# TrackieWay-OSS/TrackieLLM

Measured on AMD Instinct MI355X. Metric: cortex cycles/sec (frame+1s audio+128 tok), higher is better.
Workload: dtype int8 x q4_K/q6_K (i32 acc, f32 scales); 1 GPU; configs[3] fused cycle: YOLOv8n 640x640 frame (preprocess+network+NMS) + 1 s PCM (VAD + Whisper-tiny.en log-mel/encoder/16 forced decoder steps) + Mistral-7B Q4_K_M 64-token prefill and 128-token greedy decode, 3 concurrent HIP streams; concurrent_cycles_per_gpu=768, decode_groups=3, rows_per_llm_pass=256, layers=32, parallelism=replicas x1

## Files before the change

### trackiellm_amd/csrc/llm/tk_llm_kernels.hip

```cpp
#include "tk_llm_kernels.h"

#include "../common/tk_exact_math.h"
#include <stdio.h>
#include <stdlib.h>

#include <atomic>

#include "../common/tk_ggml_blocks.h"
#include "../common/tk_sample_device.h"

typedef int v4i __attribute__((ext_vector_type(4)));
typedef int v2i __attribute__((ext_vector_type(2)));
typedef float v4f __attribute__((ext_vector_type(4)));
typedef float v2f __attribute__((ext_vector_type(2)));

#define TK_WAVE 64

__global__ void k_synth_blocks(int type, uint64_t seed, uint64_t tid, int64_t nblocks, float scale, uint8_t* out) {
    int64_t b = (int64_t)blockIdx.x * blockDim.x + threadIdx.x;
    if (b >= nblocks) return;
    float x[256];
    for (int i = 0; i < 256; ++i) x[i] = scale * tk_synth_normal(seed, tid, (uint64_t)(256 * b + i));
    if (type == TK_TYPE_Q4_K) {
        tk_block_q4_K blk;
// ... 1436 lines not shown
    }
}

static int tk_num_cu() {
    static std::atomic<int> cached[64];
    int dev = 0;
    if (hipGetDevice(&dev) != hipSuccess || dev < 0 || dev >= 64) return 256;
    int v = cached[dev].load(std::memory_order_relaxed);
    if (v == 0) {
        int n = 0;
        v = (hipDeviceGetAttribute(&n, hipDeviceAttributeMultiprocessorCount, dev) == hipSuccess && n > 0) ? n : 256;
        cached[dev].store(v, std::memory_order_relaxed);
    }
    return v;
}
#define TK_NUM_CU tk_num_cu()

#define TK_MAX_DYN_LDS (160 * 1024)
#include <mutex>
template <typename F>
static hipError_t opt_in_lds(F* fn) { return hipFuncSetAttribute((const void*)fn, hipFuncAttributeMaxDynamicSharedMemorySize, TK_MAX_DYN_LDS); }

static constexpr int TK_GEMM32_FROM_ROWS = 12 * TK_ROW_SLOTS + 1;

typedef void (*TkGemvKernel)(TkGemvArgs, int, int);
typedef void (*TkGemm32Kernel)(TkGemvArgs, int, int, int);
static const TkGemvKernel k_gemv_fns[3][2][2][4] = {
    {{{k_gemv_w4a8<1, 1, 1, 0>, k_gemv_w4a8<1, 1, 2, 0>, k_gemv_w4a8<1, 1, 3, 0>, k_gemv_w4a8<1, 1, 4, 0>},
      {k_gemv_w4a8<2, 1, 1, 0>, k_gemv_w4a8<2, 1, 2, 0>, k_gemv_w4a8<2, 1, 3, 0>, k_gemv_w4a8<2, 1, 4, 0>}},
     {{k_gemv_w4a8<1, 2, 1, 0>, nullptr, k_gemv_w4a8<1, 2, 3, 0>, k_gemv_w4a8<1, 2, 4, 0>},
      {k_gemv_w4a8<2, 2, 1, 0>, nullptr, k_gemv_w4a8<2, 2, 3, 0>, k_gemv_w4a8<2, 2, 4, 0>}}},
    {{{}, {k_gemv_w4a8<2, 1, 1, 1>, k_gemv_w4a8<2, 1, 2, 1>, k_gemv_w4a8<2, 1, 3, 1>, k_gemv_w4a8<2, 1, 4, 1>}}},
    {{{}, {k_gemv_w4a8<2, 1, 1, 2>, k_gemv_w4a8<2, 1, 2, 2>, k_gemv_w4a8<2, 1, 3, 2>, k_gemv_w4a8<2, 1, 4, 2>}}},
};
static const TkGemvKernel k_gemm_fns[5][4] = {
    {k_gemm_w4a8<4, 1>, k_gemm_w4a8<4, 2>, k_gemm_w4a8<4, 3>, k_gemm_w4a8<4, 4>},     {k_gemm_w4a8<6, 1>, k_gemm_w4a8<6, 2>, k_gemm_w4a8<6, 3>, k_gemm_w4a8<6, 4>},
    {k_gemm_w4a8<8, 1>, k_gemm_w4a8<8, 2>, k_gemm_w4a8<8, 3>, k_gemm_w4a8<8, 4>},     {k_gemm_w4a8<10, 1>, k_gemm_w4a8<10, 2>, k_gemm_w4a8<10, 3>, k_gemm_w4a8<10, 4>},
    {k_gemm_w4a8<12, 1>, k_gemm_w4a8<12, 2>, k_gemm_w4a8<12, 3>, k_gemm_w4a8<12, 4>},
};
static const TkGemm32Kernel k_gemm32_fns[4] = {k_gemm32_w4a8<1>, k_gemm32_w4a8<2>, k_gemm32_w4a8<3>, k_gemm32_w4a8<4>};

void tk_launch_gemv(const TkGemvArgs& a, hipStream_t s) {
    int types = 0;
    for (int i = 0; i < a.nseg; ++i) types |= a.seg[i].type == TK_TYPE_Q4_K ? 1 : a.seg[i].type == TK_TYPE_Q5_K ? 4 : 2;
    if ((types & 4) && types != 4) {
        int i0 = 0, col = a.col0;
        while (i0 < a.nseg) {
            int i1 = i0 + 1;
            while (i1 < a.nseg && a.seg[i1].type == a.seg[i0].type) ++i1;
            TkGemvArgs p = a;
            p.nseg = i1 - i0;
            for (int i = 0; i < p.nseg; ++i) p.seg[i] = a.seg[i0 + i];
            p.col0 = col;
            tk_launch_gemv(p, s);
            for (int i = i0; i < i1; ++i) col += a.seg[i].row_tiles * TK_TILE_ROWS;
            i0 = i1;
        }
        return;
    }
    const int ti = types == 4 ? 3 : types - 1;
    int row_tiles = 0;
    for (int i = 0; i < a.nseg; ++i) row_tiles += a.seg[i].row_tiles;
    int groups = TK_NUM_CU / a.ks;
    if (groups < 1) groups = 1;
    if (groups > row_tiles) groups = row_tiles;
    int waves = (row_tiles + groups - 1) / groups;
    while (waves > 8) { groups *= 2; waves = (row_tiles + groups - 1) / groups; }
    if (a.nrows >= TK_GEMM32_FROM_ROWS) {
        const int pairs = a.swiglu ? a.seg[0].row_tiles : row_tiles / 2;
        const int g32 = (pairs + 3) / 4;
        const int n_halves = a.nrows > 8 * TK_ROW_SLOTS ? 2 : 1;
        const size_t ldsb = (size_t)2 * TK_G32_MT * TK_RING_TILE_BYTES;
        hipLaunchKernelGGL(k_gemm32_fns[ti], dim3(g32 * a.ks * n_halves), dim3(256), ldsb, s, a, g32, row_tiles, n_halves);
        return;
    }
    if (a.nrows > 2 * TK_ROW_SLOTS) {
        const int mtb = a.nrows > 10 * TK_ROW_SLOTS ? 12 : a.nrows > 8 * TK_ROW_SLOTS ? 10 : a.nrows > 6 * TK_ROW_SLOTS ? 8 : a.nrows > 4 * TK_ROW_SLOTS ? 6 : 4;
        const size_t ldsb = (size_t)2 * mtb * TK_RING_TILE_BYTES;
        hipLaunchKernelGGL(k_gemm_fns[mtb / 2 - 2][ti], dim3(groups * a.ks), dim3(64 * waves), ldsb, s, a, groups, row_tiles);
        return;
    }
    const int mt = a.nrows > TK_ROW_SLOTS ? 2 : 1;
    const size_t lds = tk_gemv_lds_bytes(a.K, a.ks, mt);
    const int nb = a.K / a.ks / 256;
    const int gti = mt == 2 && types == 2 ? 2 : ti;
    const int pf = nb % 2 == 0 ? 2 : 1;
    const size_t fuse_lds = a.fuse == 1 ? ((size_t)a.K + 4) * sizeof(float) : 0;
    const int fuse = a.fuse && mt == 1 && pf == 2 ? (a.fuse == 1 ? 1 : 2) : 0;
    hipLaunchKernelGGL(k_gemv_fns[fuse][mt - 1][pf - 1][gti], dim3(groups * a.ks), dim3(64 * waves), lds + fuse_lds, s, a, groups, row_tiles);
}

bool tk_gemv_fuses_producer(int nrows, int K, int ks, int fks) {
    return nrows >= 1 && nrows <= TK_GEMV_FUSE_MAX_ROWS && ks >= 1 && K % (512 * ks) == 0 && fks >= 0 && fks <= TK_RMS_MAX_KS;
}

__device__ __forceinline__ float sum_partials(const float* partial, int ks, int n_total, int row, int col) {
    float o = partial[(int64_t)row * n_total + col];
    for (int s = 1; s < ks; ++s) o = o + partial[((int64_t)s * TK_MAX_ROWS + row) * n_total + col];
    return o;
}

__global__ void k_qkv_rope_append(const float* partial, int ks, int n_total, int n_head, int n_kv_head, int head_dim, const float* rope_cos,
                                  const float* rope_sin, const int32_t* seq, const int32_t* pos, float* qbuf, uint16_t* kcache,
                                  uint16_t* vcache, int layer, int max_seq, int max_ctx) {
    const int kvh = blockIdx.x, r = blockIdx.y;
    const int half = head_dim / 2, grp = n_head / n_kv_head;
    const int QD = n_head * head_dim, KVD = n_kv_head * head_dim;
    const int p = pos[r], sq = seq[r];
    const float* cs = rope_cos + (int64_t)p * half;
    const float* sn = rope_sin + (int64_t)p * half;
    const int64_t cbase = ((((int64_t)layer * max_seq + sq) * n_kv_head + kvh) * max_ctx + p) * head_dim;
    for (int idx = threadIdx.x; idx < (grp + 1) * half; idx += blockDim.x) {
        const int hsel = idx / half, i = idx % half;
        if (hsel < grp) {
            const int col = (kvh * grp + hsel) * head_dim + 2 * i;
            const float a = sum_partials(partial, ks, n_total, r, col);
            const float b = sum_partials(partial, ks, n_total, r, col + 1);
            qbuf[(int64_t)r * QD + col] = tk_fmaf(-b, sn[i], a * cs[i]);
            qbuf[(int64_t)r * QD + col + 1] = tk_fmaf(a, sn[i], b * cs[i]);
        } else {
            const int col = QD + kvh * head_dim + 2 * i;
            const float a = sum_partials(partial, ks, n_total, r, col);
            const float b = sum_partials(partial, ks, n_total, r, col + 1);
            kcache[cbase + 2 * i] = tk_f32_to_f16(tk_fmaf(-b, sn[i], a * cs[i]));
            kcache[cbase + 2 * i + 1] = tk_f32_to_f16(tk_fmaf(a, sn[i], b * cs[i]));
            const int vcol = QD + KVD + kvh * head_dim + 2 * i;
            vcache[cbase + 2 * i] = tk_f32_to_f16(sum_partials(partial, ks, n_total, r, vcol));
            vcache[cbase + 2 * i + 1] = tk_f32_to_f16(sum_partials(partial, ks, n_total, r, vcol + 1));
        }
    }
}

void tk_launch_qkv_rope_append(const float* partial, int ks, int n_total, int n_head, int n_kv_head, int head_dim, const float* rope_cos,
                               const float* rope_sin, const int32_t* seq, const int32_t* pos, int nrows, float* qbuf, uint16_t* kcache,
                               uint16_t* vcache, int layer, int max_seq, int max_ctx, hipStream_t s) {
    hipLaunchKernelGGL(k_qkv_rope_append, dim3(n_kv_head, nrows), dim3(256), 0, s, partial, ks, n_total, n_head, n_kv_head, head_dim, rope_cos,
                       rope_sin, seq, pos, qbuf, kcache, vcache, layer, max_seq, max_ctx);
}

#define TK_ATT_MAX_GRP 4
#define TK_ATT_TSPLIT 4
__device__ __forceinline__ float sum_partials_wide(const float* partial, int ks, int n_total, int row, int col) {
    float p[TK_RMS_MAX_KS];
#pragma unroll
    for (int s = 0; s < TK_RMS_MAX_KS; ++s)
        if (s < ks) p[s] = partial[((int64_t)s * TK_MAX_ROWS + row) * n_total + col];
    float o = p[0];
#pragma unroll
    for (int s = 1; s < TK_RMS_MAX_KS; ++s)
        if (s < ks) o = o + p[s];
    return o;
}

__device__ __forceinline__ void att_stage(const uint16_t* run, int row0, int last_row, int rb , uint8_t* slot, bool swz, int wave, int lane, int chunk,
                                          int row_end = -1) {
    const int pieces = chunk * rb / 1024, ppr = rb / 16;
    for (int pc = wave; pc < pieces; pc += 4) {
        if (row_end >= 0 && row0 + pc * 64 / ppr >= row_end) continue;
        const int idx = pc * 64 + lane;
        const int r = idx / ppr, cs = idx % ppr;
        int gr = row0 + r;
        gr = gr < last_row ? gr : last_row;
        const int src = swz ? (cs ^ (r & (ppr - 1))) : cs;
        const auto gs = (const __attribute__((address_space(1))) void*)((const uint8_t*)run + (int64_t)gr * rb + src * 16);
        const auto ls = (__attribute__((address_space(3))) void*)(slot + pc * 1024);
        __builtin_amdgcn_global_load_lds(gs, ls, 16, 0, 0);
    }
}

template <int GQ, bool FUSED, int HD , int CH >
__global__ __launch_bounds__(256, 1) void k_attention(const float* __restrict__ qbuf, const float* __restrict__ partial, int ks, int n_total,
                                                    const float* __restrict__ rope_cos, const float* __restrict__ rope_sin,
                                                    uint16_t* __restrict__ kcache, uint16_t* __restrict__ vcache, const int32_t* __restrict__ seq,
                                                    const int32_t* __restrict__ pos, int n_head, int n_kv_head, int head_dim_rt, int layer, int max_seq,
                                                    int max_ctx, TkActQ8 out) {
    extern __shared__ __attribute__((aligned(16))) uint8_t att_lds[];
    const int head_dim = HD ? HD : head_dim_rt;
    const int hb = blockIdx.x, r = blockIdx.y, t = threadIdx.x, lane = t & 63;
    const int kvh = hb * GQ / (n_head / n_kv_head);
    const int wave = __builtin_amdgcn_readfirstlane(t >> 6);
    const int p = pos[r], T = p + 1, sq = seq[r];
    const int W = GQ * head_dim;
    const int rb = head_dim * 2;
    const int half = head_dim / 2, QD = n_head * head_dim, KVD = n_kv_head * head_dim;
    const int slot_bytes = CH * rb;
    uint8_t* ring = att_lds;
    float* qs = (float*)(att_lds + 2 * slot_bytes);
    float* sc = qs + W;
    float* red = sc + (size_t)GQ * max_ctx;
    uint16_t* own = (uint16_t*)(red + 4 * TK_ATT_MAX_GRP);
    float* part = (float*)ring;
    float* lpart = part + TK_ATT_TSPLIT * W;
    float* obuf = lpart + TK_ATT_TSPLIT * TK_ATT_MAX_GRP;
    const int64_t run0 = (((int64_t)layer * max_seq + sq) * n_kv_head + kvh) * (int64_t)max_ctx * head_dim;
    const uint16_t* krun = kcache + run0;
    const uint16_t* vrun = vcache + run0;
    const int nchunk = (T + CH - 1) / CH;
    const int total = 2 * nchunk;
    const int last_row = max_ctx - 1;
    const int ppr = rb / 16;
    auto issue = [&](int j) {
        const bool is_k = j < nchunk;
        const int c = is_k ? j : j - nchunk;
        att_stage(is_k ? krun : vrun, c * CH, last_row, rb, ring + (j % 2) * slot_bytes, is_k, wave, lane, CH, CH > 64 ? T : -1);
    };
    const int ppw = slot_bytes / 4096;
    auto acquire = [&](int j) {
        const int ahead = total - 1 - j < 0 ? total - 1 - j : 0;
        wait_vmcnt(ahead * ppw);
        __syncthreads();
        if (j + 1 < total) issue(j + 1);
    };

    for (int j = 0; j < 1 && j < total; ++j) issue(j);
    if (FUSED) {
        const float* cs = rope_cos + (int64_t)p * half;
        const float* sn = rope_sin + (int64_t)p * half;
        for (int idx = t; idx < (GQ + 2) * half; idx += 256) {
            const int hsel = idx / half, i = idx % half;
            if (hsel < GQ) {
                const int col = (hb * GQ + hsel) * head_dim + 2 * i;
                const float a = sum_partials_wide(partial, ks, n_total, r, col), b = sum_partials_wide(partial, ks, n_total, r, col + 1);
                qs[hsel * head_dim + 2 * i] = tk_fmaf(-b, sn[i], a * cs[i]);
                qs[hsel * head_dim + 2 * i + 1] = tk_fmaf(a, sn[i], b * cs[i]);
            } else if (hsel == GQ) {
                const int col = QD + kvh * head_dim + 2 * i;
                const float a = sum_partials_wide(partial, ks, n_total, r, col), b = sum_partials_wide(partial, ks, n_total, r, col + 1);
                const uint16_t k0 = tk_f32_to_f16(tk_fmaf(-b, sn[i], a * cs[i])), k1 = tk_f32_to_f16(tk_fmaf(a, sn[i], b * cs[i]));
                const uint32_t kk = (uint32_t)k0 | ((uint32_t)k1 << 16);
                *(uint32_t*)(kcache + run0 + (int64_t)p * head_dim + 2 * i) = kk;
                *(uint32_t*)(own + 2 * i) = kk;
            } else {
                const int col = QD + KVD + kvh * head_dim + 2 * i;
                const uint16_t v0 = tk_f32_to_f16(sum_partials_wide(partial, ks, n_total, r, col)), v1 = tk_f32_to_f16(sum_partials_wide(partial, ks, n_total, r, col + 1));
                const uint32_t vv = (uint32_t)v0 | ((uint32_t)v1 << 16);
                *(uint32_t*)(vcache + run0 + (int64_t)p * head_dim + 2 * i) = vv;
                *(uint32_t*)(own + head_dim + 2 * i) = vv;
            }
        }
    } else {
        for (int i = t; i < W; i += 256) qs[i] = qbuf[(int64_t)r * QD + hb * W + i];
    }
    const float att_scale = tk_divf(1.0f, tk_sqrtf((float)head_dim));

    float mx = -INFINITY;
    for (int c = 0; c < nchunk; ++c) {
        acquire(c);
        uint8_t* slot = ring + (c % 2) * slot_bytes;
        if (FUSED && c == nchunk - 1) {
            const int rr = p - c * CH;
            if (t < ppr) *(uint4*)(slot + rr * rb + ((t ^ (rr & (ppr - 1))) * 16)) = *(const uint4*)((const uint8_t*)own + t * 16);
            __syncthreads();
        }
        for (int idx = t; idx < GQ * CH; idx += 256) {
            const int h = idx / CH, rr = idx % CH, tt = c * CH + rr;
            if (tt < T) {
                const uint8_t* kr = slot + rr * rb;
                const float* qh = qs + h * head_dim;
                float a = 0.0f;
                constexpr int KB = HD ? HD / 8 : 1;
                for (int i0 = 0; i0 < ppr; i0 += KB) {
                    uint4 kv[KB];
#pragma unroll
                    for (int u = 0; u < KB; ++u) kv[u] = *(const uint4*)(kr + (((i0 + u) ^ (rr & (ppr - 1))) * 16));
#pragma unroll
                    for (int u = 0; u < KB; ++u) {
                        const v4f q0 = *(const v4f*)(qh + 8 * (i0 + u)), q1 = *(const v4f*)(qh + 8 * (i0 + u) + 4);
                        const uint32_t kw[4] = {kv[u].x, kv[u].y, kv[u].z, kv[u].w};
#pragma unroll
                        for (int e = 0; e < 8; ++e) {
                            const float kf = f16bits_to_f32((kw[e >> 1] >> (16 * (e & 1))) & 0xffffu);
                            a = tk_fmaf(e < 4 ? q0[e] : q1[e - 4], kf, a);
                        }
                    }
                }
                const float s = a * att_scale;
                sc[(size_t)h * max_ctx + tt] = s;
                mx = tk_fmaxf(mx, s);
            }
        }
    }
    if (CH <= 64) {
        float m = mx;
        for (int s = CH / 2; s >= 1; s >>= 1) m = tk_fmaxf(m, wave_xor_f(m, s));
        if ((lane & (CH - 1)) == 0 && t < GQ * CH) red[t / CH] = m;
    } else {
        float m = mx;
        for (int s = 32; s >= 1; s >>= 1) m = tk_fmaxf(m, wave_xor_f(m, s));
        if (lane == 0) red[TK_ATT_MAX_GRP + wave] = m;
    }
    __syncthreads();
    if (CH > 64 && t < GQ) {
        float m = red[TK_ATT_MAX_GRP + t * (CH / 64)];
        for (int w = 1; w < CH / 64; ++w) m = tk_fmaxf(m, red[TK_ATT_MAX_GRP + t * (CH / 64) + w]);
        red[t] = m;
    }
    if (CH > 64) __syncthreads();
    for (int h = 0; h < GQ; ++h) {
        const float m = red[h];
        for (int tt = t; tt < T; tt += 256) sc[(size_t)h * max_ctx + tt] = tk_expf(sc[(size_t)h * max_ctx + tt] - m);
    }
    float acc[GQ][2][2], l[GQ];
#pragma unroll
    for (int h = 0; h < GQ; ++h) { l[h] = 0.0f; acc[h][0][0] = acc[h][0][1] = acc[h][1][0] = acc[h][1][1] = 0.0f; }
    for (int c = 0; c < nchunk; ++c) {
        acquire(nchunk + c);
        uint8_t* slot = ring + ((nchunk + c) % 2) * slot_bytes;
        if (FUSED && c == nchunk - 1) {
            const int rr = p - c * CH;
            if (t < ppr) *(uint4*)(slot + rr * rb + t * 16) = *(const uint4*)((const uint8_t*)(own + head_dim) + t * 16);
            __syncthreads();
        }
        const int t_end = T - c * CH < CH ? T - c * CH : CH;
        constexpr int PB = 4;
        for (int rr0 = wave; rr0 < t_end; rr0 += PB * TK_ATT_TSPLIT) {
            float pr[PB][GQ];
            uint32_t vv[PB][2];
#pragma unroll
            for (int u = 0; u < PB; ++u) {
                const int rr = rr0 + u * TK_ATT_TSPLIT;
                const bool live = rr < t_end;
                const int rc = live ? rr : t_end - 1;
#pragma unroll
                for (int h = 0; h < GQ; ++h) pr[u][h] = live ? sc[(size_t)h * max_ctx + c * CH + rc] : 0.0f;
#pragma unroll
                for (int db = 0; db < 2; ++db) {
                    const int d0 = 2 * lane + 128 * db;
                    vv[u][db] = d0 < head_dim ? *(const uint32_t*)(slot + rc * rb + d0 * 2) : 0u;
                }
            }
#pragma unroll
            for (int u = 0; u < PB; ++u) {
#pragma unroll
                for (int db = 0; db < 2; ++db) {
                    if (2 * lane + 128 * db < head_dim) {
                        const float v0 = f16bits_to_f32(vv[u][db] & 0xffffu), v1 = f16bits_to_f32(vv[u][db] >> 16);
#pragma unroll
                        for (int h = 0; h < GQ; ++h) {
                            acc[h][db][0] = tk_fmaf(pr[u][h], v0, acc[h][db][0]);
                            acc[h][db][1] = tk_fmaf(pr[u][h], v1, acc[h][db][1]);
                        }
                    }
                }
#pragma unroll
                for (int h = 0; h < GQ; ++h) l[h] = l[h] + pr[u][h];
            }
        }
    }
    __syncthreads();
#pragma unroll
    for (int h = 0; h < GQ; ++h) {
#pragma unroll
        for (int db = 0; db < 2; ++db) {
            const int d0 = 2 * lane + 128 * db;
            if (d0 < head_dim) {
                part[wave * W + h * head_dim + d0] = acc[h][db][0];
                part[wave * W + h * head_dim + d0 + 1] = acc[h][db][1];
            }
        }
        if (lane == 0) lpart[wave * TK_ATT_MAX_GRP + h] = l[h];
    }
    __syncthreads();
    for (int i = t; i < W; i += 256) {
        const int h = i / head_dim;
        const float a = ((part[i] + part[W + i]) + part[2 * W + i]) + part[3 * W + i];
        const float ll = ((lpart[h] + lpart[TK_ATT_MAX_GRP + h]) + lpart[2 * TK_ATT_MAX_GRP + h]) + lpart[3 * TK_ATT_MAX_GRP + h];
        obuf[i] = tk_divf(a, ll);
    }
    __syncthreads();
    for (int c = t; c < W / 8; c += 256) {
        float v[8];
#pragma unroll
        for (int i = 0; i < 8; ++i) v[i] = obuf[8 * c + i];
        quantize_chunk8(v, hb * (W / 8) + c, r, out);
    }
}

__global__ __launch_bounds__(1024) void k_attention_narrow(const float* __restrict__ partial, int ks, int n_total, const float* __restrict__ rope_cos,
                                                            const float* __restrict__ rope_sin, uint16_t* __restrict__ kcache, uint16_t* __restrict__ vcache,
                                                            const int32_t* __restrict__ seq, const int32_t* __restrict__ pos, int n_head, int n_kv_head, int layer,
                                                            int max_seq, int max_ctx, int cap, TkActQ8 out) {
    extern __shared__ __attribute__((aligned(16))) uint8_t att_lds[];
    constexpr int HD = 128, GQ = 2, W = GQ * HD, RB = HD * 2, PPR = RB / 16;
    const int hb = blockIdx.x, r = blockIdx.y, t = threadIdx.x, lane = t & 63;
    const int wave = __builtin_amdgcn_readfirstlane(t >> 6);
    const int kvh = hb * GQ / (n_head / n_kv_head);
    const int p = pos[r], T = p + 1, sq = seq[r];
    const int half = HD / 2, QD = n_head * HD, KVD = n_kv_head * HD;
    uint8_t* kbuf = att_lds;
    uint8_t* vbuf = att_lds + (size_t)cap * RB;
    float* qs = (float*)(att_lds + (size_t)2 * cap * RB);
    float* sc = qs + W;
    float* red = sc + (size_t)GQ * ((max_ctx + 3) & ~3);
    uint16_t* own = (uint16_t*)(red + 32);
    float* part = (float*)kbuf;
    float* lpart = part + TK_ATT_TSPLIT * W;
    float* obuf = lpart + TK_ATT_TSPLIT * TK_ATT_MAX_GRP;
    const int64_t run0 = (((int64_t)layer * max_seq + sq) * n_kv_head + kvh) * (int64_t)max_ctx * HD;
    const int nchunk = (T + cap - 1) / cap;
    auto stage = [&](const uint16_t* run, int row0, uint8_t* buf, bool swz) {
        const int pieces = cap * RB / 1024;
        for (int pc = wave; pc < pieces; pc += 16) {
            if (row0 + pc * 4 >= T) break;
            const int rr = pc * 4 + (lane >> 4), cs = lane & 15;
            int gr = row0 + rr;
            gr = gr < max_ctx - 1 ? gr : max_ctx - 1;
            const int src = swz ? (cs ^ (rr & (PPR - 1))) : cs;
            const auto gs = (const __attribute__((address_space(1))) void*)((const uint8_t*)run + (int64_t)gr * RB + src * 16);
            const auto ls = (__attribute__((address_space(3))) void*)(buf + pc * 1024);
            __builtin_amdgcn_global_load_lds(gs, ls, 16, 0, 0);
        }
    };
    stage(kcache + run0, 0, kbuf, true);
    stage(vcache + run0, 0, vbuf, false);
    if (t < (GQ + 2) * half) {
        const float* cs = rope_cos + (int64_t)p * half;
        const float* sn = rope_sin + (int64_t)p * half;
        const int hsel = t / half, i = t % half;
        if (hsel < GQ) {
            const int col = (hb * GQ + hsel) * HD + 2 * i;
            const float a = sum_partials_wide(partial, ks, n_total, r, col), b = sum_partials_wide(partial, ks, n_total, r, col + 1);
            qs[hsel * HD + 2 * i] = tk_fmaf(-b, sn[i], a * cs[i]);
            qs[hsel * HD + 2 * i + 1] = tk_fmaf(a, sn[i], b * cs[i]);
        } else if (hsel == GQ) {
            const int col = QD + kvh * HD + 2 * i;
            const float a = sum_partials_wide(partial, ks, n_total, r, col), b = sum_partials_wide(partial, ks, n_total, r, col + 1);
            const uint16_t k0 = tk_f32_to_f16(tk_fmaf(-b, sn[i], a * cs[i])), k1 = tk_f32_to_f16(tk_fmaf(a, sn[i], b * cs[i]));
            const uint32_t kk = (uint32_t)k0 | ((uint32_t)k1 << 16);
            if ((hb * GQ) % (n_head / n_kv_head) == 0) *(uint32_t*)(kcache + run0 + (int64_t)p * HD + 2 * i) = kk;
            *(uint32_t*)(own + 2 * i) = kk;
        } else {
            const int col = QD + KVD + kvh * HD + 2 * i;
            const uint16_t v0 = tk_f32_to_f16(sum_partials_wide(partial, ks, n_total, r, col)), v1 = tk_f32_to_f16(sum_partials_wide(partial, ks, n_total, r, col + 1));
            const uint32_t vv = (uint32_t)v0 | ((uint32_t)v1 << 16);
            if ((hb * GQ) % (n_head / n_kv_head) == 0) *(uint32_t*)(vcache + run0 + (int64_t)p * HD + 2 * i) = vv;
            *(uint32_t*)(own + HD + 2 * i) = vv;
        }
    }
    const float att_scale = tk_divf(1.0f, tk_sqrtf((float)HD));
    const int sh = wave & 1;
    float mx = -INFINITY;
    for (int c = 0; c < nchunk; ++c) {
        if (c > 0) { __syncthreads(); stage(kcache + run0, c * cap, kbuf, true); }
        __builtin_amdgcn_s_waitcnt(0x0F70);
        __syncthreads();
        if (c == nchunk - 1) {
            const int rr = p - c * cap;
            if (t < PPR) *(uint4*)(kbuf + rr * RB + ((t ^ (rr & (PPR - 1))) * 16)) = *(const uint4*)((const uint8_t*)own + t * 16);
            if (t >= 64 && t < 64 + PPR && nchunk == 1) *(uint4*)(vbuf + rr * RB + (t - 64) * 16) = *(const uint4*)((const uint8_t*)(own + HD) + (t - 64) * 16);
            __syncthreads();
        }
        const int tc = T - c * cap < cap ? T - c * cap : cap;
        for (int rr = (wave >> 1) * 64 + lane; rr < tc; rr += 512) {
            const uint8_t* kr = kbuf + rr * RB;
            const float* qh = qs + sh * HD;
            uint4 kv[PPR];
#pragma unroll
            for (int u = 0; u < PPR; ++u) kv[u] = *(const uint4*)(kr + ((u ^ (rr & (PPR - 1))) * 16));
            float a = 0.0f;
#pragma unroll
            for (int u = 0; u < PPR; ++u) {
                const v4f q0 = *(const v4f*)(qh + 8 * u), q1 = *(const v4f*)(qh + 8 * u + 4);
                const uint32_t kw[4] = {kv[u].x, kv[u].y, kv[u].z, kv[u].w};
#pragma unroll
                for (int e = 0; e < 8; ++e) {
                    const float kf = f16bits_to_f32((kw[e >> 1] >> (16 * (e & 1))) & 0xffffu);
                    a = tk_fmaf(e < 4 ? q0[e] : q1[e - 4], kf, a);
                }
            }
            const float sv = a * att_scale;
            sc[(size_t)sh * max_ctx + c * cap + rr] = sv;
            mx = tk_fmaxf(mx, sv);
        }
    }
    for (int s2 = 32; s2 >= 1; s2 >>= 1) mx = tk_fmaxf(mx, wave_xor_f(mx, s2));
    if (lane == 0) red[wave] = mx;
    __syncthreads();
// ... 415 lines not shown
        }
#pragma unroll
        for (int k = 0; k < 32; ++k) {
            int tt = j + 4 * (32 * c + k);
            tt = tt < T ? tt : T - 1;
            v[k] = *(const uint32_t*)(vrun + (int64_t)tt * HD + 2 * dl);
        }
    };
    auto score_of = [&](int c) -> float {
        const int i = 32 * c + (lane & 31);
        return i < nj ? s[j + 4 * i] : -INFINITY;
    };
    auto probs = [&](float sc, int c) -> float { return 32 * c + (lane & 31) < nj ? tk_expf(sc - m) : 0.0f; };
    __shared__ float ebuf[2][32];
    int eslot = 0;
    auto eat = [&](const uint32_t (&v)[32], float e32) {
        if (lane < 32) ebuf[eslot][lane] = e32;
        __syncthreads();
        float ek[32];
#pragma unroll
        for (int k = 0; k < 32; ++k) ek[k] = ebuf[eslot][k];
        eslot ^= 1;
#pragma unroll
        for (int k = 0; k < 32; ++k) {
            acc0 = tk_fmaf(ek[k], f16bits_to_f32(v[k] & 0xffffu), acc0);
            acc1 = tk_fmaf(ek[k], f16bits_to_f32(v[k] >> 16), acc1);
            l = l + ek[k];
        }
    };
    const int nch = (nj + 31) / 32;
    float sa = score_of(0), sb = score_of(1);
    if (nch > 0) fetch(va, 0);
    for (int c = 0; c < nch; c += 2) {
        const float ea = probs(sa, c);
        sa = score_of(c + 2);
        fetch(vb, c + 1);
        eat(va, ea);
        if (c + 1 >= nch) break;
        const float eb = probs(sb, c + 1);
        sb = score_of(c + 3);
        if (c + 2 < nch) fetch(va, c + 2);
        eat(vb, eb);
    }
    float* pp = pv_part + (((int64_t)r * n_head + head) * TK_ATT_TSPLIT + j) * HD;
    if (lane < HD / 2) { pp[2 * dl] = acc0; pp[2 * dl + 1] = acc1; }
    if (lane == 0) l_part[((int64_t)r * n_head + head) * TK_ATT_TSPLIT + j] = l;
}

template <int HD>
__global__ __launch_bounds__(256) void k_att_pv_join(const float* __restrict__ pv_part, const float* __restrict__ l_part, int n_head, TkActQ8 out) {
    __shared__ float obuf[256];
    constexpr int HPB = 256 / HD;
    const int r = blockIdx.y, t = threadIdx.x;
    const int head = blockIdx.x * HPB + t / HD, dd = t % HD;
    const float* pp = pv_part + ((int64_t)r * n_head + head) * TK_ATT_TSPLIT * HD + dd;
    const float* lp = l_part + ((int64_t)r * n_head + head) * TK_ATT_TSPLIT;
    const float a = ((pp[0] + pp[HD]) + pp[2 * HD]) + pp[3 * HD];
    const float ll = ((lp[0] + lp[1]) + lp[2]) + lp[3];
    obuf[t] = tk_divf(a, ll);
    __syncthreads();
    if (t < 32) {
        float v[8];
#pragma unroll
        for (int i = 0; i < 8; ++i) v[i] = obuf[8 * t + i];
        quantize_chunk8(v, blockIdx.x * 32 + t, r, out);
    }
}

void tk_launch_attention_long(const float* partial, int ks, int n_total, const float* rope_cos, const float* rope_sin, uint16_t* kcache, uint16_t* vcache,
                              const int32_t* seq, const int32_t* pos, int nrows, int n_head, int n_kv_head, int head_dim, int layer, int max_seq, int max_ctx,
                              float* scores, TkActQ8 out, hipStream_t s) {
    const dim3 gs(n_kv_head, (max_ctx + 63) / 64, nrows);
    float* pv_part = scores + (size_t)TK_LONG_ATT_MAX_ROWS * n_head * max_ctx;
    float* l_part = pv_part + (size_t)TK_LONG_ATT_MAX_ROWS * n_head * TK_ATT_TSPLIT * head_dim;
    const dim3 gc(TK_ATT_TSPLIT, n_head, nrows);
    if (head_dim == 128) {
        hipLaunchKernelGGL((k_att_scores_long<128>), gs, dim3(256), 0, s, partial, ks, n_total, rope_cos, rope_sin, kcache, vcache, seq, pos, n_head, n_kv_head, layer,
                           max_seq, max_ctx, scores);
        hipLaunchKernelGGL((k_att_pv_chain<128>), gc, dim3(64), 0, s, scores, vcache, seq, pos, n_head, n_kv_head, layer, max_seq, max_ctx, pv_part, l_part);
        hipLaunchKernelGGL((k_att_pv_join<128>), dim3(n_head / 2, nrows), dim3(256), 0, s, pv_part, l_part, n_head, out);
    } else {
        hipLaunchKernelGGL((k_att_scores_long<64>), gs, dim3(256), 0, s, partial, ks, n_total, rope_cos, rope_sin, kcache, vcache, seq, pos, n_head, n_kv_head, layer,
                           max_seq, max_ctx, scores);
        hipLaunchKernelGGL((k_att_pv_chain<64>), gc, dim3(64), 0, s, scores, vcache, seq, pos, n_head, n_kv_head, layer, max_seq, max_ctx, pv_part, l_part);
        hipLaunchKernelGGL((k_att_pv_join<64>), dim3(n_head / 4, nrows), dim3(256), 0, s, pv_part, l_part, n_head, out);
    }
}

size_t tk_attention_long_scratch_floats(int n_head, int head_dim, int max_ctx) {
    return (size_t)TK_LONG_ATT_MAX_ROWS * n_head * ((size_t)max_ctx + (size_t)TK_ATT_TSPLIT * head_dim + TK_ATT_TSPLIT);
}

bool tk_attention_long_applies(int nrows, int n_head, int n_kv_head, int head_dim) {
    const char* np = getenv("TK_MI355X_NO_LONG_ATT");
    if (np && np[0] == '1') return false;
    if (nrows < 1 || nrows > TK_LONG_ATT_MAX_ROWS || (head_dim != 64 && head_dim != 128)) return false;
    const int hpb = 256 / head_dim, grp = n_kv_head > 0 ? n_head / n_kv_head : 0;
    return grp >= 1 && grp <= 4 && grp % hpb == 0 && n_head % hpb == 0;
}

bool tk_attention_prefill_applies(int n_head, int n_kv_head, int head_dim) {
    const char* np = getenv("TK_MI355X_NO_PREFILL_ATT");
    if (np && np[0] == '1') return false;
    if (head_dim != 64 && head_dim != 128) return false;
    const int hpb = 256 / head_dim, grp = n_kv_head > 0 ? n_head / n_kv_head : 0;
    return grp > 0 && grp % hpb == 0 && n_head % hpb == 0;
}

void tk_launch_att_tiles(const int32_t* seq, int nrows, int32_t* tiles, hipStream_t s) {
    hipLaunchKernelGGL(k_att_tiles, dim3(1), dim3(TK_MAX_ROWS), 0, s, seq, nrows, tiles);
}

void tk_launch_attention_prefill(const float* qbuf, const uint16_t* kcache, const uint16_t* vcache, const int32_t* seq, const int32_t* pos,
                                 const int32_t* tiles, int nrows, int n_head, int n_kv_head, int head_dim, int layer, int max_seq, int max_ctx, TkActQ8 out,
                                 hipStream_t s) {
    if (head_dim == 128)
        hipLaunchKernelGGL((k_attention_prefill<128>), dim3(n_head / 2, nrows / 16 + 8), dim3(512), TkPrefillLds<128>::bytes, s, qbuf, kcache, vcache, seq, pos, tiles, n_head,
                           n_kv_head, layer, max_seq, max_ctx, out);
    else
        hipLaunchKernelGGL((k_attention_prefill<64>), dim3(n_head / 4, nrows / 16 + 8), dim3(1024), TkPrefillLds<64>::bytes, s, qbuf, kcache, vcache, seq, pos, tiles, n_head,
                           n_kv_head, layer, max_seq, max_ctx, out);
}

static size_t tk_attention_narrow_fixed_lds(int max_ctx) {
    return (size_t)(2 * 128 + 2 * (size_t)((max_ctx + 3) & ~3) + 32) * sizeof(float) + 2 * 128 * 2;
}
static std::atomic<int> g_sessions_alive[64];
void tk_attention_note_session(int device, int delta) {
    if (device >= 0 && device < 64) g_sessions_alive[device].fetch_add(delta, std::memory_order_relaxed);
}
static bool tk_device_is_shared_by_sessions() {
    int dev = 0;
    if (hipGetDevice(&dev) != hipSuccess || dev < 0 || dev >= 64) return false;
    return g_sessions_alive[dev].load(std::memory_order_relaxed) > 1;
}
static int tk_attention_narrow_cap(int nrows, int n_head, int n_kv_head, int head_dim, int max_ctx, bool fused) {
    const int grp = n_kv_head > 0 ? n_head / n_kv_head : 0;
    if (!fused || head_dim != 128 || (grp != 2 && grp != 4) || (n_head / 2) * nrows > TK_NUM_CU) return 0;
    const char* nn = getenv("TK_MI355X_NO_NARROW_ATT");
    if (nn && nn[0] == '1') return 0;
    if (!(nn && nn[0] == '0') && tk_device_is_shared_by_sessions()) return 0;
    const size_t fixed = tk_attention_narrow_fixed_lds(max_ctx);
    if (fixed + 64 * 512 > (size_t)TK_MAX_DYN_LDS) return 0;
    int cap = (int)(((size_t)TK_MAX_DYN_LDS - fixed) / 512);
    const int want = (max_ctx + 31) / 32 * 32;
    cap = cap > want ? want : cap;
    return cap / 32 * 32;
}

size_t tk_attention_lds_bytes(int gq, int head_dim, int max_ctx, int chunk) {
    const size_t W = (size_t)gq * head_dim;
    const size_t ring = (size_t)2 * chunk * head_dim * 2;
    const size_t epilogue = ((size_t)TK_ATT_TSPLIT * W + TK_ATT_TSPLIT * TK_ATT_MAX_GRP + W) * sizeof(float);
    return (ring > epilogue ? ring : epilogue) + (W + (size_t)gq * max_ctx + 4 * TK_ATT_MAX_GRP) * sizeof(float) + (size_t)2 * head_dim * 2;
}

TkAttentionPlan tk_attention_plan(int nrows, int n_head, int n_kv_head, int head_dim, int max_ctx, bool fused) {
    TkAttentionPlan pl{};
    if (const int cap = tk_attention_narrow_cap(nrows, n_head, n_kv_head, head_dim, max_ctx, fused)) {
        pl.kernel = 1; pl.gq = 2; pl.chunk = cap; pl.slots = 1;
        pl.lds_bytes = tk_attention_narrow_fixed_lds(max_ctx) + (size_t)cap * 512;
        return pl;
    }
    int gq = n_head / n_kv_head;
    if (gq == 4 && (2 * head_dim) % 256 == 0 && nrows * n_kv_head < 2 * TK_NUM_CU) gq = 2;
    const bool narrow = gq * 128 <= 256 && (n_head / gq) * nrows <= TK_NUM_CU && (head_dim == 128 || head_dim == 64) &&
                        tk_attention_lds_bytes(gq, head_dim, max_ctx, 128) <= (size_t)TK_MAX_DYN_LDS;
    const int chunk = narrow ? 128 : (n_head / gq) * nrows > 4 * TK_NUM_CU ? 32 : 64;
    pl.kernel = 0; pl.gq = gq; pl.chunk = chunk; pl.slots = 2;
    pl.lds_bytes = tk_attention_lds_bytes(gq, head_dim, max_ctx, chunk);
    if (!fused && tk_attention_prefill_applies(n_head, n_kv_head, head_dim)) pl.kernel = 2;
    return pl;
}

typedef void (*TkAttentionKernel)(const float*, const float*, int, int, const float*, const float*, uint16_t*, uint16_t*, const int32_t*,
                                  const int32_t*, int, int, int, int, int, int, TkActQ8);
static const TkAttentionKernel k_attention_fns[3][2][3][3] = {
    {{{k_attention<1, false, 0, 32>, k_attention<1, false, 0, 64>},
      {k_attention<1, false, 64, 32>, k_attention<1, false, 64, 64>, k_attention<1, false, 64, 128>},
      {k_attention<1, false, 128, 32>, k_attention<1, false, 128, 64>, k_attention<1, false, 128, 128>}},
     {{k_attention<1, true, 0, 32>, k_attention<1, true, 0, 64>},
      {k_attention<1, true, 64, 32>, k_attention<1, true, 64, 64>, k_attention<1, true, 64, 128>},
      {k_attention<1, true, 128, 32>, k_attention<1, true, 128, 64>, k_attention<1, true, 128, 128>}}},
    {{{k_attention<2, false, 0, 32>, k_attention<2, false, 0, 64>},
      {k_attention<2, false, 64, 32>, k_attention<2, false, 64, 64>, k_attention<2, false, 64, 128>},
      {k_attention<2, false, 128, 32>, k_attention<2, false, 128, 64>, k_attention<2, false, 128, 128>}},
     {{k_attention<2, true, 0, 32>, k_attention<2, true, 0, 64>},
      {k_attention<2, true, 64, 32>, k_attention<2, true, 64, 64>, k_attention<2, true, 64, 128>},
      {k_attention<2, true, 128, 32>, k_attention<2, true, 128, 64>, k_attention<2, true, 128, 128>}}},
    {{{k_attention<4, false, 0, 32>, k_attention<4, false, 0, 64>},
      {k_attention<4, false, 64, 32>, k_attention<4, false, 64, 64>},
      {k_attention<4, false, 128, 32>, k_attention<4, false, 128, 64>}},
     {{k_attention<4, true, 0, 32>, k_attention<4, true, 0, 64>},
      {k_attention<4, true, 64, 32>, k_attention<4, true, 64, 64>},
      {k_attention<4, true, 128, 32>, k_attention<4, true, 128, 64>}}},
};

void tk_launch_attention(const float* qbuf, const float* partial, int ks, int n_total, const float* rope_cos, const float* rope_sin,
                         uint16_t* kcache, uint16_t* vcache, const int32_t* seq, const int32_t* pos, int nrows, int n_head, int n_kv_head,
                         int head_dim, int layer, int max_seq, int max_ctx, TkActQ8 out, bool fused, hipStream_t s) {
    const TkAttentionPlan pl = tk_attention_plan(nrows, n_head, n_kv_head, head_dim, max_ctx, fused);
    if (pl.kernel == 1) {
        hipLaunchKernelGGL(k_attention_narrow, dim3(n_head / 2, nrows), dim3(1024), pl.lds_bytes, s, partial, ks, n_total, rope_cos, rope_sin, kcache,
                           vcache, seq, pos, n_head, n_kv_head, layer, max_seq, max_ctx, pl.chunk, out);
        return;
    }
    const int gq = pl.gq, chunk = pl.chunk;
    const TkAttentionKernel k = k_attention_fns[gq == 4 ? 2 : gq - 1][fused][head_dim == 128 ? 2 : head_dim == 64 ? 1 : 0][chunk == 128 ? 2 : chunk == 64 ? 1 : 0];
    hipLaunchKernelGGL(k, dim3(n_head / gq, nrows), dim3(256), pl.lds_bytes, s, qbuf, partial, ks, n_total, rope_cos, rope_sin, kcache, vcache, seq, pos,
                       n_head, n_kv_head, head_dim, layer, max_seq, max_ctx, out);
}

template <int KSM>
__global__ __launch_bounds__(256) void k_swiglu_q8(const float* partial, int ks, int FF, TkActQ8 out) {
    const int r = blockIdx.y;
    const int c = blockIdx.x * 256 + threadIdx.x;
    if (c >= FF / 8) return;
    v4f g[2], u[2];
    {
        v4f pg[KSM][2], pu[KSM][2];
#pragma unroll
        for (int s = 0; s < KSM; ++s)
            if (s < ks) {
                const float* row = partial + ((int64_t)s * TK_MAX_ROWS + r) * (2 * (int64_t)FF);
                pg[s][0] = *(const v4f*)(row + 8 * c); pg[s][1] = *(const v4f*)(row + 8 * c + 4);
                pu[s][0] = *(const v4f*)(row + FF + 8 * c); pu[s][1] = *(const v4f*)(row + FF + 8 * c + 4);
            }
        g[0] = pg[0][0]; g[1] = pg[0][1]; u[0] = pu[0][0]; u[1] = pu[0][1];
#pragma unroll
        for (int s = 1; s < KSM; ++s)
            if (s < ks) { g[0] = g[0] + pg[s][0]; g[1] = g[1] + pg[s][1]; u[0] = u[0] + pu[s][0]; u[1] = u[1] + pu[s][1]; }
    }
    float v[8];
#pragma unroll
    for (int i = 0; i < 8; ++i) v[i] = tk_siluf(g[i >> 2][i & 3]) * u[i >> 2][i & 3];
    quantize_chunk8(v, c, r, out);
}

__global__ __launch_bounds__(256) void k_quant_q8(const float* __restrict__ hbuf, int FF, TkActQ8 out) {
    const int r = blockIdx.y;
    const int c = blockIdx.x * 256 + threadIdx.x;
    if (c >= FF / 8) return;
    const float* row = hbuf + (int64_t)r * FF + 8 * c;
    const v4f a = *(const v4f*)row, b = *(const v4f*)(row + 4);
    float v[8] = {a[0], a[1], a[2], a[3], b[0], b[1], b[2], b[3]};
    quantize_chunk8(v, c, r, out);
}

void tk_launch_quant_q8(const float* hbuf, int FF, int nrows, TkActQ8 out, hipStream_t s) {
    hipLaunchKernelGGL(k_quant_q8, dim3((FF / 8 + 255) / 256, nrows), dim3(256), 0, s, hbuf, FF, out);
}

bool tk_gemv_fuses_swiglu(int nrows, int ks, int type_gate, int type_up) {
    return nrows >= TK_GEMM32_FROM_ROWS && ks == 1 && type_gate == type_up &&
           (type_gate == TK_TYPE_Q4_K || type_gate == TK_TYPE_Q5_K || type_gate == TK_TYPE_Q6_K);
}

void tk_launch_swiglu_q8(const float* partial, int ks, int FF, int nrows, TkActQ8 out, hipStream_t s) {
    if (ks == 1) hipLaunchKernelGGL((k_swiglu_q8<1>), dim3((FF / 8 + 255) / 256, nrows), dim3(256), 0, s, partial, ks, FF, out);
    else hipLaunchKernelGGL((k_swiglu_q8<TK_RMS_MAX_KS>), dim3((FF / 8 + 255) / 256, nrows), dim3(256), 0, s, partial, ks, FF, out);
}

__global__ __launch_bounds__(1024) void k_argmax(const float* logits, int vocab, const uint32_t* allow_base, const int32_t* allow_row, TkSampleRow* samp,
                                                  int32_t* tok, int32_t* pos, int32_t* nsteps, int32_t* hist, int hist_stride) {
    __shared__ float bv[16];
    __shared__ int bi[16];
    __shared__ uint32_t sm[256 + 8 + 4 * TK_SAMPLE_MAX_K];
    const int r = blockIdx.x, t = threadIdx.x;
    const float* lg = logits + (int64_t)r * vocab;
    const int mi = allow_row ? allow_row[r] : -1;
    const uint32_t* allow = mi >= 0 ? allow_base + (size_t)mi * ((vocab + 31) / 32) : nullptr;
    float best = -INFINITY;
    int idx = 0x7fffffff;
    if (samp && samp[r].temp > 0.0f) {
        __shared__ int32_t picked;
        const TkSampleRow sp = samp[r];
        sample_row(lg, vocab, allow, sp, &picked, sm);
        __syncthreads();
        if (t == 0) { idx = picked; samp[r].counter = sp.counter + 1; }
    } else {
    constexpr int NU = 8;
    if (allow) {
        for (int i0 = t; i0 < vocab; i0 += 1024 * NU) {
            float v[NU];
            uint32_t m[NU];
#pragma unroll
            for (int u = 0; u < NU; ++u) {
                const int i = i0 + 1024 * u, ic = i < vocab ? i : vocab - 1;
                v[u] = lg[ic];
                m[u] = allow[ic >> 5];
            }
#pragma unroll
            for (int u = 0; u < NU; ++u) {
                const int i = i0 + 1024 * u;
                if (i < vocab && ((m[u] >> (i & 31)) & 1u) && (v[u] > best || idx == 0x7fffffff)) { best = v[u]; idx = i; }
            }
        }
    } else {
        for (int i0 = t; i0 < vocab; i0 += 1024 * NU) {
            float v[NU];
#pragma unroll
            for (int u = 0; u < NU; ++u) {
                const int i = i0 + 1024 * u;
                v[u] = lg[i < vocab ? i : vocab - 1];
            }
#pragma unroll
            for (int u = 0; u < NU; ++u) {
// ... 55 lines not shown
```

Before: 180.1 cycles/s.

## Restructure decode attention LDS layout and score pass to raise occupancy

Reworks the decode attention kernel so that q and the first score chunks alias the score buffer, shrinking dynamic LDS, and raises the launch-bounds waves-per-EU hint so more blocks can be resident. K chunks are now processed in reverse order so the early chunks stay in registers and are written back after the q buffer is dead. Scores are stored token-major so the PV loop reads a head group with one vector load. Partial-sum reduction loads adjacent column pairs as v2f, and the own V row is kept in a register instead of LDS. The double-buffer prefetch now waits for all outstanding loads, which may reduce overlap, and the aliasing makes correctness depend on careful ordering.

```diff
diff --git a/trackiellm_amd/csrc/llm/tk_llm_kernels.hip b/trackiellm_amd/csrc/llm/tk_llm_kernels.hip
--- a/trackiellm_amd/csrc/llm/tk_llm_kernels.hip
+++ b/trackiellm_amd/csrc/llm/tk_llm_kernels.hip
@@ -1612,6 +1612,22 @@
     return o;
 }
 
+__device__ __forceinline__ v2f sum_partials_pair(const float* partial, int ks, int n_total, int row, int col) {
+    const int64_t slab = (int64_t)TK_MAX_ROWS * n_total;
+    const float* base = partial + (int64_t)row * n_total;
+    v2f o = *(const v2f*)(base + (uint32_t)col);
+    for (int s0 = 1; s0 < ks; s0 += 3) {
+        v2f q[3];
+#pragma unroll
+        for (int u = 0; u < 3; ++u)
+            if (s0 + u < ks) q[u] = *(const v2f*)(base + (s0 + u) * slab + (uint32_t)col);
+#pragma unroll
+        for (int u = 0; u < 3; ++u)
+            if (s0 + u < ks) o = o + q[u];
+    }
+    return o;
+}
+
 __device__ __forceinline__ void att_stage(const uint16_t* run, int row0, int last_row, int rb , uint8_t* slot, bool swz, int wave, int lane, int chunk,
                                           int row_end = -1) {
     const int pieces = chunk * rb / 1024, ppr = rb / 16;
@@ -1629,7 +1645,7 @@
 }
 
 template <int GQ, bool FUSED, int HD , int CH >
-__global__ __launch_bounds__(256, 1) void k_attention(const float* __restrict__ qbuf, const float* __restrict__ partial, int ks, int n_total,
+__global__ __launch_bounds__(256, CH == 32 ? 8 : 4) void k_attention(const float* __restrict__ qbuf, const float* __restrict__ partial, int ks, int n_total,
                                                     const float* __restrict__ rope_cos, const float* __restrict__ rope_sin,
                                                     uint16_t* __restrict__ kcache, uint16_t* __restrict__ vcache, const int32_t* __restrict__ seq,
                                                     const int32_t* __restrict__ pos, int n_head, int n_kv_head, int head_dim_rt, int layer, int max_seq,
@@ -1644,11 +1660,13 @@
     const int rb = head_dim * 2;
     const int half = head_dim / 2, QD = n_head * head_dim, KVD = n_kv_head * head_dim;
     const int slot_bytes = CH * rb;
+    constexpr int NH = HD ? (HD + CH - 1) / CH : 0;
+    const int scp = HD && max_ctx < HD + HD / 2 ? HD + HD / 2 : max_ctx;
     uint8_t* ring = att_lds;
-    float* qs = (float*)(att_lds + 2 * slot_bytes);
-    float* sc = qs + W;
-    float* red = sc + (size_t)GQ * max_ctx;
-    uint16_t* own = (uint16_t*)(red + 4 * TK_ATT_MAX_GRP);
+    float* sc = (float*)(att_lds + 2 * slot_bytes);
+    float* qs = HD ? sc : sc + (size_t)GQ * scp;
+    float* red = HD ? sc + (size_t)GQ * scp : qs + W;
+    uint16_t* own = HD ? (uint16_t*)(sc + W) : (uint16_t*)(red + (CH > 64 ? 4 * TK_ATT_MAX_GRP : 0));
     float* part = (float*)ring;
     float* lpart = part + TK_ATT_TSPLIT * W;
     float* obuf = lpart + TK_ATT_TSPLIT * TK_ATT_MAX_GRP;
@@ -1661,41 +1679,38 @@
     const int ppr = rb / 16;
     auto issue = [&](int j) {
         const bool is_k = j < nchunk;
-        const int c = is_k ? j : j - nchunk;
+        const int c = is_k ? nchunk - 1 - j : j - nchunk;
         att_stage(is_k ? krun : vrun, c * CH, last_row, rb, ring + (j % 2) * slot_bytes, is_k, wave, lane, CH, CH > 64 ? T : -1);
     };
-    const int ppw = slot_bytes / 4096;
     auto acquire = [&](int j) {
-        const int ahead = total - 1 - j < 0 ? total - 1 - j : 0;
-        wait_vmcnt(ahead * ppw);
+        wait_vmcnt(0);
         __syncthreads();
         if (j + 1 < total) issue(j + 1);
     };
 
-    for (int j = 0; j < 1 && j < total; ++j) issue(j);
+    issue(0);
+    uint32_t own_v = 0;
+    const int own_vi = (t + 256 * (((GQ + 1) * half - t + 255) / 256)) - (GQ + 1) * half;
     if (FUSED) {
         const float* cs = rope_cos + (int64_t)p * half;
         const float* sn = rope_sin + (int64_t)p * half;
         for (int idx = t; idx < (GQ + 2) * half; idx += 256) {
             const int hsel = idx / half, i = idx % half;
+            const int col = (hsel < GQ ? (hb * GQ + hsel) * head_dim : hsel == GQ ? QD + kvh * head_dim : QD + KVD + kvh * head_dim) + 2 * i;
+            const v2f ab = sum_partials_pair(partial, ks, n_total, r, col);
+            const float a = ab[0], b = ab[1];
             if (hsel < GQ) {
-                const int col = (hb * GQ + hsel) * head_dim + 2 * i;
-                const float a = sum_partials_wide(partial, ks, n_total, r, col), b = sum_partials_wide(partial, ks, n_total, r, col + 1);
                 qs[hsel * head_dim + 2 * i] = tk_fmaf(-b, sn[i], a * cs[i]);
                 qs[hsel * head_dim + 2 * i + 1] = tk_fmaf(a, sn[i], b * cs[i]);
             } else if (hsel == GQ) {
-                const int col = QD + kvh * head_dim + 2 * i;
-                const float a = sum_partials_wide(partial, ks, n_total, r, col), b = sum_partials_wide(partial, ks, n_total, r, col + 1);
                 const uint16_t k0 = tk_f32_to_f16(tk_fmaf(-b, sn[i], a * cs[i])), k1 = tk_f32_to_f16(tk_fmaf(a, sn[i], b * cs[i]));
                 const uint32_t kk = (uint32_t)k0 | ((uint32_t)k1 << 16);
                 *(uint32_t*)(kcache + run0 + (int64_t)p * head_dim + 2 * i) = kk;
                 *(uint32_t*)(own + 2 * i) = kk;
             } else {
-                const int col = QD + KVD + kvh * head_dim + 2 * i;
-                const uint16_t v0 = tk_f32_to_f16(sum_partials_wide(partial, ks, n_total, r, col)), v1 = tk_f32_to_f16(sum_partials_wide(partial, ks, n_total, r, col + 1));
-                const uint32_t vv = (uint32_t)v0 | ((uint32_t)v1 << 16);
+                const uint32_t vv = (uint32_t)tk_f32_to_f16(a) | ((uint32_t)tk_f32_to_f16(b) << 16);
                 *(uint32_t*)(vcache + run0 + (int64_t)p * head_dim + 2 * i) = vv;
-                *(uint32_t*)(own + head_dim + 2 * i) = vv;
+                own_v = vv;
             }
         }
     } else {
@@ -1703,62 +1718,72 @@
     }
     const float att_scale = tk_divf(1.0f, tk_sqrtf((float)head_dim));
 
+    const bool scorer = t < GQ * CH;
+    const int sh = t / CH, srr = t % CH;
     float mx = -INFINITY;
-    for (int c = 0; c < nchunk; ++c) {
-        acquire(c);
-        uint8_t* slot = ring + (c % 2) * slot_bytes;
-        if (FUSED && c == nchunk - 1) {
+    float held[NH ? NH : 1];
+#pragma unroll
+    for (int u = 0; u < (NH ? NH : 1); ++u) held[u] = 0.0f;
+    for (int j = 0; j < nchunk; ++j) {
+        const int c = nchunk - 1 - j;
+        acquire(j);
+        uint8_t* slot = ring + (j % 2) * slot_bytes;
+        if (FUSED && j == 0) {
             const int rr = p - c * CH;
             if (t < ppr) *(uint4*)(slot + rr * rb + ((t ^ (rr & (ppr - 1))) * 16)) = *(const uint4*)((const uint8_t*)own + t * 16);
             __syncthreads();
         }
-        for (int idx = t; idx < GQ * CH; idx += 256) {
-            const int h = idx / CH, rr = idx % CH, tt = c * CH + rr;
-            if (tt < T) {
-                const uint8_t* kr = slot + rr * rb;
-                const float* qh = qs + h * head_dim;
-                float a = 0.0f;
-                constexpr int KB = HD ? HD / 8 : 1;
-                for (int i0 = 0; i0 < ppr; i0 += KB) {
-                    uint4 kv[KB];
-#pragma unroll
-                    for (int u = 0; u < KB; ++u) kv[u] = *(const uint4*)(kr + (((i0 + u) ^ (rr & (ppr - 1))) * 16));
-#pragma unroll
-                    for (int u = 0; u < KB; ++u) {
-                        const v4f q0 = *(const v4f*)(qh + 8 * (i0 + u)), q1 = *(const v4f*)(qh + 8 * (i0 + u) + 4);
-                        const uint32_t kw[4] = {kv[u].x, kv[u].y, kv[u].z, kv[u].w};
-#pragma unroll
-                        for (int e = 0; e < 8; ++e) {
-                            const float kf = f16bits_to_f32((kw[e >> 1] >> (16 * (e & 1))) & 0xffffu);
-                            a = tk_fmaf(e < 4 ? q0[e] : q1[e - 4], kf, a);
-                        }
+        const int tt = c * CH + srr;
+        if (scorer && tt < T) {
+            const uint8_t* kr = slot + srr * rb;
+            const float* qh = qs + sh * head_dim;
+            float a = 0.0f;
+            constexpr int KB = HD ? HD / 8 : 1;
+            for (int i0 = 0; i0 < ppr; i0 += KB) {
+                uint4 kv[KB];
+#pragma unroll
+                for (int u = 0; u < KB; ++u) kv[u] = *(const uint4*)(kr + (((i0 + u) ^ (srr & (ppr - 1))) * 16));
+#pragma unroll
+                for (int u = 0; u < KB; ++u) {
+                    const v4f q0 = *(const v4f*)(qh + 8 * (i0 + u)), q1 = *(const v4f*)(qh + 8 * (i0 + u) + 4);
+                    const uint32_t kw[4] = {kv[u].x, kv[u].y, kv[u].z, kv[u].w};
+#pragma unroll
+                    for (int e = 0; e < 8; ++e) {
+                        const float kf = f16bits_to_f32((kw[e >> 1] >> (16 * (e & 1))) & 0xffffu);
+                        a = tk_fmaf(e < 4 ? q0[e] : q1[e - 4], kf, a);
                     }
                 }
-                const float s = a * att_scale;
-                sc[(size_t)h * max_ctx + tt] = s;
-                mx = tk_fmaxf(mx, s);
-            }
-        }
-    }
+            }
+            const float s = a * att_scale;
+            mx = tk_fmaxf(mx, s);
+            if (c >= NH) sc[(size_t)tt * GQ + sh] = s;
+#pragma unroll
+            for (int u = 0; u < NH; ++u) held[u] = c == u ? s : held[u];
+        }
+    }
+    float m = mx;
     if (CH <= 64) {
-        float m = mx;
         for (int s = CH / 2; s >= 1; s >>= 1) m = tk_fmaxf(m, wave_xor_f(m, s));
-        if ((lane & (CH - 1)) == 0 && t < GQ * CH) red[t / CH] = m;
     } else {
-        float m = mx;
         for (int s = 32; s >= 1; s >>= 1) m = tk_fmaxf(m, wave_xor_f(m, s));
         if (lane == 0) red[TK_ATT_MAX_GRP + wave] = m;
-    }
-    __syncthreads();
-    if (CH > 64 && t < GQ) {
-        float m = red[TK_ATT_MAX_GRP + t * (CH / 64)];
-        for (int w = 1; w < CH / 64; ++w) m = tk_fmaxf(m, red[TK_ATT_MAX_GRP + t * (CH / 64) + w]);
-        red[t] = m;
-    }
-    if (CH > 64) __syncthreads();
-    for (int h = 0; h < GQ; ++h) {
-        const float m = red[h];
-        for (int tt = t; tt < T; tt += 256) sc[(size_t)h * max_ctx + tt] = tk_expf(sc[(size_t)h * max_ctx + tt] - m);
+        __syncthreads();
+        if (t < GQ) {
+            float mm = red[TK_ATT_MAX_GRP + t * (CH / 64)];
+            for (int w = 1; w < CH / 64; ++w) mm = tk_fmaxf(mm, red[TK_ATT_MAX_GRP + t * (CH / 64) + w]);
+            red[t] = mm;
+        }
+        __syncthreads();
+        m = red[scorer ? sh : 0];
+    }
+    if (scorer) {
+        for (int c = NH; c < nchunk; ++c) {
+            const int tt = c * CH + srr;
+            if (tt < T) sc[(size_t)tt * GQ + sh] = tk_expf(sc[(size_t)tt * GQ + sh] - m);
+        }
+#pragma unroll
+        for (int u = 0; u < NH; ++u)
+            if (u * CH + srr < T) held[u] = tk_expf(held[u] - m);
     }
     float acc[GQ][2][2], l[GQ];
 #pragma unroll
@@ -1766,9 +1791,17 @@
     for (int c = 0; c < nchunk; ++c) {
         acquire(nchunk + c);
         uint8_t* slot = ring + ((nchunk + c) % 2) * slot_bytes;
+        if (c == 0 && NH) {
+            if (scorer) {
+#pragma unroll
+                for (int u = 0; u < NH; ++u)
+                    if (u * CH + srr < T) sc[(size_t)(u * CH + srr) * GQ + sh] = held[u];
+            }
+            if (!(FUSED && c == nchunk - 1)) __syncthreads();
+        }
         if (FUSED && c == nchunk - 1) {
             const int rr = p - c * CH;
-            if (t < ppr) *(uint4*)(slot + rr * rb + t * 16) = *(const uint4*)((const uint8_t*)(own + head_dim) + t * 16);
+            if (own_vi < half) *(uint32_t*)(slot + rr * rb + own_vi * 4) = own_v;
             __syncthreads();
         }
         const int t_end = T - c * CH < CH ? T - c * CH : CH;
@@ -1781,8 +1814,12 @@
                 const int rr = rr0 + u * TK_ATT_TSPLIT;
                 const bool live = rr < t_end;
                 const int rc = live ? rr : t_end - 1;
-#pragma unroll
-                for (int h = 0; h < GQ; ++h) pr[u][h] = live ? sc[(size_t)h * max_ctx + c * CH + rc] : 0.0f;
+                const float* pp = sc + (size_t)(c * CH + rc) * GQ;
+                if (GQ == 4) { const v4f x = *(const v4f*)pp; pr[u][0] = x[0]; pr[u][1 % GQ] = x[1]; pr[u][2 % GQ] = x[2]; pr[u][3 % GQ] = x[3]; }
+                else if (GQ == 2) { const v2f x = *(const v2f*)pp; pr[u][0] = x[0]; pr[u][1 % GQ] = x[1]; }
+                else pr[u][0] = pp[0];
+#pragma unroll
+                for (int h = 0; h < GQ; ++h) pr[u][h] = live ? pr[u][h] : 0.0f;
 #pragma unroll
                 for (int db = 0; db < 2; ++db) {
                     const int d0 = 2 * lane + 128 * db;
@@ -2504,7 +2541,12 @@
     const size_t W = (size_t)gq * head_dim;
     const size_t ring = (size_t)2 * chunk * head_dim * 2;
     const size_t epilogue = ((size_t)TK_ATT_TSPLIT * W + TK_ATT_TSPLIT * TK_ATT_MAX_GRP + W) * sizeof(float);
-    return (ring > epilogue ? ring : epilogue) + (W + (size_t)gq * max_ctx + 4 * TK_ATT_MAX_GRP) * sizeof(float) + (size_t)2 * head_dim * 2;
+    const size_t red = chunk > 64 ? 4 * TK_ATT_MAX_GRP * sizeof(float) : 0;
+    if (head_dim == 128 || head_dim == 64) {
+        const size_t scp = max_ctx > head_dim + head_dim / 2 ? max_ctx : head_dim + head_dim / 2;
+        return (ring > epilogue ? ring : epilogue) + (size_t)gq * scp * sizeof(float) + red;
+    }
+    return (ring > epilogue ? ring : epilogue) + ((size_t)gq * max_ctx + W) * sizeof(float) + red + (size_t)head_dim * 2;
 }
 
 TkAttentionPlan tk_attention_plan(int nrows, int n_head, int n_kv_head, int head_dim, int max_ctx, bool fused) {
```

Measured after the change: 183.8 cycles/s (median of 6 runs). +2.1%, better.
